# raphaelsulzer/PixelsPointsPolygons

Hardware: NVIDIA B200
Metric: pillar_encode_tiles_per_sec (higher is better)
Workload: dtype f16 operands, f32 accumulate, f32 in/out

## Files before the change

### pixelspointspolygons_b200/csrc/pfn.cu

```cuda
#include <cuda_fp16.h>

#include "p3p_internal.cuh"

namespace p3p {

#ifdef P3P_TIMELINE
constexpr int kTlCtas = 4, kTlRoles = 12, kTlIters = 96, kTlStamps = 4;
__device__ long long g_pfn_tl[kTlCtas][kTlRoles][kTlIters][kTlStamps];
__device__ __forceinline__ void ptl(int role, long long it, int k) {
    if ((threadIdx.x & 31) == 0 && blockIdx.x < kTlCtas && it < kTlIters) g_pfn_tl[blockIdx.x][role][it][k] = clock64();
}
#define PTL(role, it, k) ptl(role, it, k)
extern "C" int p3p_debug_pfn_timeline(long long* host) {
    return (int)cudaMemcpyFromSymbol(host, g_pfn_tl, sizeof(g_pfn_tl));
}
#else
#define PTL(role, it, k)
#endif

void make_blob_layout(int C, BlobLayout* out) {
    BlobLayout l;
    l.C = C;
    l.Cpad = (C + 127) / 128 * 128;
    l.MT = l.Cpad / 128;
    size_t off = 0;
    auto take = [&](size_t bytes) {
        size_t o = off;
        off += (bytes + 1023) / 1024 * 1024;
        return o;
    };
    l.off_header = take(64);
    l.off_front = take(10 * 32 * 4);
    l.off_w0 = take(32 * 8 * 4);
    l.off_b0 = take(32 * 4);
    l.off_w1 = take((size_t)l.Cpad * 64 * 4);
    l.off_b1 = take((size_t)l.Cpad * 4);
    l.off_a1 = take((size_t)l.Cpad * 128);
    l.off_a2 = take((size_t)l.Cpad * 128);
    l.total_bytes = off;
    *out = l;
}

namespace {

__global__ void pfn_prepare_kernel(p3p_pfn_params p, int precision, char* blob, BlobLayout bl) {
    const int tid = blockIdx.x * blockDim.x + threadIdx.x;
    const int nthreads = gridDim.x * blockDim.x;
    int* header = reinterpret_cast<int*>(blob + bl.off_header);
    float* front = reinterpret_cast<float*>(blob + bl.off_front);
    float* w0 = reinterpret_cast<float*>(blob + bl.off_w0);
    float* b0 = reinterpret_cast<float*>(blob + bl.off_b0);
    float* w1 = reinterpret_cast<float*>(blob + bl.off_w1);
    float* b1 = reinterpret_cast<float*>(blob + bl.off_b1);
    if (tid == 0) {
        header[0] = kBlobMagic; header[1] = precision; header[2] = bl.C; header[3] = bl.Cpad; header[4] = p.center_alias;
    }
    for (int k = tid; k < kC0; k += nthreads) {
        const float a = p.norm0_weight[k] / sqrtf(p.norm0_var[k] + p.eps);
        const float sh = p.norm0_bias[k] - p.norm0_mean[k] * a;
        float w[8];
        for (int i = 0; i < 8; ++i) {
            w[i] = a * p.linear0_weight[k * 8 + i];
            w0[k * 8 + i] = w[i];
        }
        b0[k] = sh;
        front[0 * 32 + k] = w[0] + w[3] + w[6];
        front[1 * 32 + k] = w[1] + w[4] + w[7];
        front[2 * 32 + k] = w[2] + w[5];
        front[3 * 32 + k] = p.center_alias ? 0.f : w[0];
        front[4 * 32 + k] = p.center_alias ? 0.f : w[1];
        front[5 * 32 + k] = w[3];
        front[6 * 32 + k] = w[4];
        front[7 * 32 + k] = w[5];
        front[8 * 32 + k] = sh;
        front[9 * 32 + k] = fmaxf(sh, 0.f);
        if (precision == P3P_PRECISION_TF32) {
            const float up = 1.0f + 0x1p-12f;
            for (int r = 0; r < 10; ++r) front[r * 32 + k] *= up;
        }
    }
    const bool tf32 = (precision != P3P_PRECISION_BF16 && precision != P3P_PRECISION_FP16);
    for (int c = tid; c < bl.Cpad; c += nthreads) {
        float a = 0.f, sh = 0.f;
        if (c < bl.C) {
            a = p.norm1_weight[c] / sqrtf(p.norm1_var[c] + p.eps);
            sh = p.norm1_bias[c] - p.norm1_mean[c] * a;
        }
        b1[c] = sh;
        const int t = c >> 7, r = c & 127;
        for (int j = 0; j < 64; ++j) {
            const float v = (c < bl.C) ? a * p.linear1_weight[c * 64 + j] : 0.f;
            w1[c * 64 + j] = v;
            const int k = j & 31;
            char* tile = blob + (j < 32 ? bl.off_a1 : bl.off_a2);
            if (tf32) {
                const size_t o = (size_t)t * 16384 + (size_t)(r >> 3) * 1024 + (size_t)(r & 7) * 128 +
                                 (size_t)(((k >> 2) ^ (r & 7)) * 16) + (size_t)(k & 3) * 4;
                *reinterpret_cast<uint32_t*>(tile + o) = to_tf32(v);
            } else {
                const size_t o = (size_t)t * 8192 + (size_t)(r >> 3) * 512 + (size_t)(r & 7) * 64 +
                                 (size_t)(((k >> 3) ^ ((r >> 1) & 3)) * 16) + (size_t)(k & 7) * 2;
                *reinterpret_cast<unsigned short*>(tile + o) = (precision == P3P_PRECISION_FP16)
                                                                   ? __half_as_ushort(__float2half_rn(v))
                                                                   : (unsigned short)(pack_bf16(v, 0.f) & 0xFFFF);
            }
        }
    }
}

__device__ __forceinline__ void store_scalar(const PfnArgs& a, int64_t idx, float v) {
    if (a.out_dtype == P3P_DTYPE_F32) {
        static_cast<float*>(a.out)[idx] = v;
    } else {
        static_cast<unsigned short*>(a.out)[idx] = to_16bit(v, a.out_dtype);
    }
}
__device__ __forceinline__ int64_t out_index(const PfnArgs& a, int64_t item, int b, int cell, int c) {
    if (a.item_mode == kItemsCanvas && a.out_layout == P3P_LAYOUT_NCHW)
        return ((int64_t)b * a.c_total + a.c_offset + c) * a.items_per_tile + cell;
    return item * a.row_stride + a.row_offset + c;
}
__device__ __forceinline__ void store_item(const PfnArgs& a, int64_t item, int b, int cell, int c, float v) {
    if (a.token_rows) {
        static_cast<float*>(a.out)[((int64_t)b * a.token_rows + 1 + cell) * a.bl.C + c] = v + a.pos_embed[(int64_t)(1 + cell) * a.bl.C + c];
        return;
    }
    store_scalar(a, out_index(a, item, b, cell, c), v);
}

constexpr int kSimtMaxThreads = 512;
constexpr int kHStride = 36;

template <bool kHoist>
__global__ void __launch_bounds__(kSimtMaxThreads) pfn_simt_kernel(PfnArgs a) {
    extern __shared__ __align__(16) float smem_f[];
    float* H = smem_f;
    float* w0s = H + (size_t)(a.g.M + 1) * kHStride;
    float* b0s = w0s + 256;
    int* red = reinterpret_cast<int*>(b0s + 32);
    int* hmax_bits = red + 96;

    const int tid = threadIdx.x, lane = tid & 31, w = tid >> 5, nthreads = blockDim.x, nwarps = nthreads >> 5;
    const float* w0g = reinterpret_cast<const float*>(a.blob + a.bl.off_w0);
    const float* b0g = reinterpret_cast<const float*>(a.blob + a.bl.off_b0);
    const float* w1g = reinterpret_cast<const float*>(a.blob + a.bl.off_w1);
    const float* b1g = reinterpret_cast<const float*>(a.blob + a.bl.off_b1);
    const int alias = reinterpret_cast<const int*>(a.blob + a.bl.off_header)[4];
    for (int i = tid; i < 256; i += nthreads) w0s[i] = w0g[i];
    if (tid < 32) b0s[tid] = b0g[tid];
    const int C = a.bl.C, M = a.g.M;
    float wa[32], wb[32], b1c = 0.f;
    if (kHoist) {
        const int c = tid < C ? tid : 0;
        b1c = b1g[c];
#pragma unroll
        for (int k = 0; k < 32; ++k) { wa[k] = w1g[(size_t)c * 64 + k]; wb[k] = w1g[(size_t)c * 64 + 32 + k]; }
    }
    __syncthreads();

    for (int64_t item = blockIdx.x; item < a.num_items; item += gridDim.x) {
        const Item it = fetch_item(a, item);
        if (!it.valid) {
            if (a.item_mode == kItemsCanvas)
                for (int c = tid; c < C; c += nthreads) store_item(a, item, it.b, it.cell, c, 0.f);
            continue;
        }
        const float4* slot = item_slots(a, it);
        const int n = it.n;
        int sl[3] = {0, 0, 0}, sh[3] = {0, 0, 0};
        for (int r = tid; r < n; r += nthreads) {
            const float4 p = slot[r];
            int lo, hi;
            fix_split(p.x, a.g.fix_scale, lo, hi); sl[0] += lo; sh[0] += hi;
            fix_split(p.y, a.g.fix_scale, lo, hi); sl[1] += lo; sh[1] += hi;
            fix_split(p.z, a.g.fix_scale, lo, hi); sl[2] += lo; sh[2] += hi;
        }
#pragma unroll
        for (int i = 0; i < 3; ++i) {
            sl[i] = __reduce_add_sync(0xffffffffu, sl[i]);
            sh[i] = __reduce_add_sync(0xffffffffu, sh[i]);
            if (lane == 0) { red[w * 6 + i] = sl[i]; red[w * 6 + 3 + i] = sh[i]; }
        }
        if (tid < 32) hmax_bits[tid] = 0;
        __syncthreads();
        int tl[3] = {0, 0, 0}, th[3] = {0, 0, 0};
        for (int ww = 0; ww < nwarps; ++ww) {
#pragma unroll
            for (int i = 0; i < 3; ++i) { tl[i] += red[ww * 6 + i]; th[i] += red[ww * 6 + 3 + i]; }
        }
        const float fn = (float)n;
        const float mx = fix_mean(tl[0], th[0], a.g.fix_inv, fn);
        const float my = fix_mean(tl[1], th[1], a.g.fix_inv, fn);
        const float mz = fix_mean(tl[2], th[2], a.g.fix_inv, fn);

        float hm[32];
#pragma unroll
        for (int k = 0; k < 32; ++k) hm[k] = 0.f;
        bool any_row = false;
        for (int r = tid; r < n; r += nthreads) {
            any_row = true;
            const float4 p = slot[r];
            float d[8];
            const float xc = p.x - it.ctr_x, yc = p.y - it.ctr_y;
            d[0] = alias ? xc : p.x; d[1] = alias ? yc : p.y; d[2] = p.z;
            d[3] = p.x - mx; d[4] = p.y - my; d[5] = p.z - mz;
            d[6] = xc; d[7] = yc;
            float* hrow = H + (size_t)r * kHStride;
#pragma unroll
            for (int k = 0; k < 32; ++k) {
                float acc = 0.f;
#pragma unroll
                for (int i = 0; i < 8; ++i) acc = __fmaf_rn(w0s[k * 8 + i], d[i], acc);
                const float h = fmaxf(acc + b0s[k], 0.f);
                hrow[k] = h;
                hm[k] = fmaxf(hm[k], h);
            }
        }
        if (__any_sync(0xffffffffu, any_row)) {
#pragma unroll
            for (int k = 0; k < 32; ++k) {
                const float v = warp_max_f32(hm[k]);
                if (lane == 0) atomicMax(&hmax_bits[k], __float_as_int(v));
            }
        }
        if (n < M && tid < 32) {
            const float hp = fmaxf(b0s[tid], 0.f);
            H[(size_t)n * kHStride + tid] = hp;
            atomicMax(&hmax_bits[tid], __float_as_int(hp));
        }
        __syncthreads();
        const int rows = n + (n < M ? 1 : 0);
        if (kHoist) {
            if (tid < C) {
                float g = b1c;
#pragma unroll
                for (int k = 0; k < 32; ++k) g = __fmaf_rn(wb[k], __int_as_float(hmax_bits[k]), g);
                float best = -INFINITY;
                for (int r = 0; r < rows; ++r) {
                    const float4* hr = reinterpret_cast<const float4*>(H + (size_t)r * kHStride);
                    float acc = 0.f;
#pragma unroll
                    for (int k4 = 0; k4 < 8; ++k4) {
                        const float4 h = hr[k4];
                        acc = __fmaf_rn(wa[k4 * 4 + 0], h.x, acc);
                        acc = __fmaf_rn(wa[k4 * 4 + 1], h.y, acc);
                        acc = __fmaf_rn(wa[k4 * 4 + 2], h.z, acc);
                        acc = __fmaf_rn(wa[k4 * 4 + 3], h.w, acc);
                    }
                    best = fmaxf(best, acc);
                }
                store_item(a, item, it.b, it.cell, tid, fmaxf(best + g, 0.f));
            }
        } else {
            for (int c = tid; c < C; c += nthreads) {
                float g = b1g[c];
#pragma unroll
                for (int k = 0; k < 32; ++k) {
                    wa[k] = w1g[(size_t)c * 64 + k];
                    g = __fmaf_rn(w1g[(size_t)c * 64 + 32 + k], __int_as_float(hmax_bits[k]), g);
                }
                float best = -INFINITY;
                for (int r = 0; r < rows; ++r) {
                    const float4* hr = reinterpret_cast<const float4*>(H + (size_t)r * kHStride);
                    float acc = 0.f;
#pragma unroll
                    for (int k4 = 0; k4 < 8; ++k4) {
                        const float4 h = hr[k4];
                        acc = __fmaf_rn(wa[k4 * 4 + 0], h.x, acc);
                        acc = __fmaf_rn(wa[k4 * 4 + 1], h.y, acc);
                        acc = __fmaf_rn(wa[k4 * 4 + 2], h.z, acc);
                        acc = __fmaf_rn(wa[k4 * 4 + 3], h.w, acc);
                    }
                    best = fmaxf(best, acc);
                }
                store_item(a, item, it.b, it.cell, c, fmaxf(best + g, 0.f));
            }
        }
        __syncthreads();
    }
}

__global__ void cls_rows_kernel(PfnArgs a, const float* __restrict__ cls_token) {
    const int C = a.bl.C;
    const int64_t total = (int64_t)a.B * C;
    for (int64_t i = (int64_t)blockIdx.x * blockDim.x + threadIdx.x; i < total; i += (int64_t)gridDim.x * blockDim.x) {
        const int64_t b = i / C;
        const int c = (int)(i - b * C);
        static_cast<float*>(a.out)[b * a.token_rows * C + c] = cls_token[c] + a.pos_embed[c];
    }
}

__global__ void zero_lidar_kernel(PfnArgs a) {
    const int C = a.bl.C;
    const int64_t total = a.num_items * C;
    for (int64_t i = (int64_t)blockIdx.x * blockDim.x + threadIdx.x; i < total; i += (int64_t)gridDim.x * blockDim.x) {
        int64_t idx;
        if (a.out_layout == P3P_LAYOUT_NCHW) {
            const int64_t per_tile = (int64_t)C * a.items_per_tile;
            const int64_t b = i / per_tile, rem = i - b * per_tile;
            idx = (b * a.c_total + a.c_offset) * a.items_per_tile + rem;
        } else {
            const int64_t item = i / C;
            idx = item * a.row_stride + a.row_offset + (i - item * C);
        }
        store_scalar(a, idx, 0.f);
    }
}

constexpr int kNF = 8;
constexpr int kMmaWarps = 4;
constexpr int kEpiWarp0 = kMmaWarps + kNF;
constexpr int kEpiGroups = 3;
constexpr int kTcThreads = 32 * (kEpiWarp0 + 4 * kEpiGroups);

constexpr int kRegMma = 40, kRegFront = 104, kRegEpi = 72;
static_assert(4 * kRegMma + 8 * kRegFront + 12 * kRegEpi <= 24 * 80, "register pool of the launch exceeded");
constexpr int kUnit = 8;
constexpr int kPairsPerUnit = kUnit / 2;
constexpr int kTiles = 3;
constexpr int kAccCols = 64;
constexpr int kAccStages = 2;
constexpr int kGCol0 = kTiles * kAccStages * kAccCols;
constexpr int kGSlotCols = kTiles * 16;
constexpr int kValidRing = 64;
constexpr int kStageRows = 128;

template <int kPrec>
struct TcCfg {
    static constexpr bool kTf32 = (kPrec == P3P_PRECISION_TF32);
    static constexpr int kFmt = kTf32 ? 2 : (kPrec == P3P_PRECISION_BF16 ? 1 : 0);
    static constexpr int RB = kTf32 ? 128 : 64;
    static constexpr int kATile = 128 * RB;
    static constexpr int kHStage = kStageRows * RB;
    static constexpr int kGStage = 16 * RB;
    static constexpr uint32_t kLayout = kTf32 ? 2u : 4u;
    static constexpr uint32_t kSBO = 8 * RB;
    static constexpr int kKSteps = kTf32 ? 4 : 2;
    static constexpr int kNS = kTf32 ? 4 : 8;
    static constexpr size_t kSmemOperands = (size_t)6 * kATile + (size_t)kNS * kHStage + 2 * (size_t)kGStage;
    static constexpr size_t kSmemFloats = 10 * 32 + 384 + kNF * 128 * 4;
    static constexpr size_t kSmemBytes = kSmemOperands + kSmemFloats * 4 + (2 * kNS + 2 * kTiles * kAccStages + 4 * kTiles + 2 + 2) * 8 + 16 + 2 * kNF * 4 + 2 * kValidRing + 4 * kEpiGroups * kUnit * 32 * 4 + 2 * kNF * 4 * 4 + 2 * kNF * 32 * 4;
};


template <int kPrec>
__device__ __forceinline__ uint32_t pack_relu16(float lo, float hi) {
    uint32_t r;
    if constexpr (kPrec == P3P_PRECISION_BF16)
        asm("cvt.rn.relu.bf16x2.f32 %0, %1, %2;" : "=r"(r) : "f"(hi), "f"(lo));
    else
        asm("cvt.rn.relu.f16x2.f32 %0, %1, %2;" : "=r"(r) : "f"(hi), "f"(lo));
    return r;
}
template <int kPrec>
__device__ __forceinline__ uint32_t max16x2(uint32_t a, uint32_t b) {
    uint32_t r;
    if constexpr (kPrec == P3P_PRECISION_BF16)
        asm("max.bf16x2 %0, %1, %2;" : "=r"(r) : "r"(a), "r"(b));
    else
        asm("max.f16x2 %0, %1, %2;" : "=r"(r) : "r"(a), "r"(b));
    return r;
}
__device__ __forceinline__ void sts128(uint32_t addr, uint32_t a, uint32_t b, uint32_t c, uint32_t d) {
    asm volatile("st.shared.v4.b32 [%0], {%1, %2, %3, %4};" ::"r"(addr), "r"(a), "r"(b), "r"(c), "r"(d) : "memory");
}
__device__ __forceinline__ void cp_async16(uint32_t dst, const void* src, uint32_t src_bytes) {
    asm volatile("cp.async.ca.shared.global [%0], [%1], 16, %2;" ::"r"(dst), "l"(src), "r"(src_bytes) : "memory");
}
template <int kRegs>
__device__ __forceinline__ void setmaxnreg_inc() { asm volatile("setmaxnreg.inc.sync.aligned.u32 %0;" ::"n"(kRegs)); }
template <int kRegs>
__device__ __forceinline__ void setmaxnreg_dec() { asm volatile("setmaxnreg.dec.sync.aligned.u32 %0;" ::"n"(kRegs)); }
__device__ __forceinline__ void cp_async4(uint32_t dst, const void* src) {
    asm volatile("cp.async.ca.shared.global [%0], [%1], 4;" ::"r"(dst), "l"(src) : "memory");
}
__device__ __forceinline__ void cp_async_wait_all() { asm volatile("cp.async.wait_all;" ::: "memory"); }

struct ItemWalk {
    int b, r, ipt, db, dr;
    __device__ __forceinline__ void init(int item, int delta, int items_per_tile) {
        ipt = items_per_tile;
        b = item / ipt; r = item - b * ipt;
        db = delta / ipt; dr = delta - db * ipt;
    }
    __device__ __forceinline__ void step() {
        b += db; r += dr;
        if (r >= ipt) { r -= ipt; ++b; }
    }
};

__device__ __forceinline__ void tmem_ld8_wait(uint32_t taddr, float (&v)[8]) {
    asm volatile(
        "tcgen05.ld.sync.aligned.32x32b.x8.b32 {%0,%1,%2,%3,%4,%5,%6,%7}, [%8];\n"
        "tcgen05.wait::ld.sync.aligned;\n"
        : "=f"(v[0]), "=f"(v[1]), "=f"(v[2]), "=f"(v[3]), "=f"(v[4]), "=f"(v[5]), "=f"(v[6]), "=f"(v[7])
        : "r"(taddr)
        : "memory");
}
__device__ __forceinline__ float max16(const float (&v)[16]) {
    float r[5];
#pragma unroll
    for (int i = 0; i < 5; ++i) r[i] = fmax3(v[3 * i], v[3 * i + 1], v[3 * i + 2]);
    return fmax3(fmax3(r[0], r[1], r[2]), fmaxf(r[3], r[4]), v[15]);
}
__device__ __forceinline__ float max16_with(float prev, const float (&v)[16]) {
    const float r0 = fmax3(prev, v[0], v[1]), r1 = fmax3(v[2], v[3], v[4]), r2 = fmax3(v[5], v[6], v[7]);
    const float r3 = fmax3(v[8], v[9], v[10]), r4 = fmax3(v[11], v[12], v[13]);
    return fmax3(fmax3(r0, r1, r2), fmax3(r3, r4, v[14]), v[15]);
}
template <int kPrec, int kMode>
__global__ void __launch_bounds__(kTcThreads, 1) pfn_tc_kernel(PfnArgs a) {
    using Cfg = TcCfg<kPrec>;
    constexpr bool kTf32 = Cfg::kTf32;
    constexpr int kNS = Cfg::kNS;
    extern __shared__ __align__(1024) unsigned char smem_dyn[];
    unsigned char* base = smem_dyn;
    unsigned char* sA1 = base;
    unsigned char* sA2 = sA1 + 3 * Cfg::kATile;
    unsigned char* sH = sA2 + 3 * Cfg::kATile;
    unsigned char* sG = sH + kNS * Cfg::kHStage;
    float* sFront = reinterpret_cast<float*>(sG + 2 * Cfg::kGStage);
    float* sB1 = sFront + 10 * 32;
    float4* sPts = reinterpret_cast<float4*>(sB1 + 384);
    uint64_t* bars = reinterpret_cast<uint64_t*>(sPts + kNF * 128);
    uint64_t* h_full = bars;
    uint64_t* h_empty = bars + kNS;
    uint64_t* t_full = bars + 2 * kNS;
    uint64_t* t_empty = t_full + kTiles * kAccStages;
    uint64_t* gt_full = t_empty + kTiles * kAccStages;
    uint64_t* gt_empty = gt_full + 2 * kTiles;
    uint64_t* g_empty = gt_empty + 2 * kTiles;
    uint32_t* tmem_slot = reinterpret_cast<uint32_t*>(g_empty + 2);
    int* sDesc = reinterpret_cast<int*>(tmem_slot + 2);
    unsigned char* sValid = reinterpret_cast<unsigned char*>(sDesc + 2 * kNF);
    float* sRmax = reinterpret_cast<float*>(sValid + 2 * kValidRing);
    int* sBlkSum = reinterpret_cast<int*>(sRmax + 4 * kEpiGroups * kUnit * 32);
    uint32_t* sBlkMax = reinterpret_cast<uint32_t*>(sBlkSum + 2 * kNF * 4);

    const int tid = threadIdx.x, warp = tid >> 5, lane = tid & 31;
    const int MT = a.bl.MT;
    const int total_items = (int)a.num_items;
    const int bs = (kMode == 0) ? a.blk_shift : 0;
    const int num_units = ((total_items << bs) + kUnit - 1) / kUnit;
    const int my_units = (num_units > (int)blockIdx.x) ? (num_units - (int)blockIdx.x + (int)gridDim.x - 1) / (int)gridDim.x : 0;
    const int my_pairs = my_units * kPairsPerUnit;
    const bool canvas = (kMode != 0) || (a.item_mode == kItemsCanvas);

    if ((smem_u32(smem_dyn) & 1023u) != 0u) __trap();
    if (warp == 0) tmem_alloc(tmem_slot, 512);
    if (tid == 32) {
        for (int i = 0; i < kNS; ++i) { mbar_init(&h_full[i], 2); mbar_init(&h_empty[i], (uint32_t)MT); }
        for (int i = 0; i < kTiles * kAccStages; ++i) { mbar_init(&t_full[i], 1); mbar_init(&t_empty[i], 128); }
        for (int i = 0; i < 2 * kTiles; ++i) { mbar_init(&gt_full[i], 1); mbar_init(&gt_empty[i], 128); }
        mbar_init(&g_empty[0], (uint32_t)MT); mbar_init(&g_empty[1], (uint32_t)MT);
        fence_mbar_init();
    }
    {
        const uint4* g1 = reinterpret_cast<const uint4*>(a.blob + a.bl.off_a1);
        const uint4* g2 = reinterpret_cast<const uint4*>(a.blob + a.bl.off_a2);
        const int nvec = MT * Cfg::kATile / 16;
        for (int i = tid; i < nvec; i += kTcThreads) {
            reinterpret_cast<uint4*>(sA1)[i] = g1[i];
            reinterpret_cast<uint4*>(sA2)[i] = g2[i];
        }
        for (int i = tid; i < 2 * Cfg::kGStage / 16; i += kTcThreads) reinterpret_cast<uint4*>(sG)[i] = make_uint4(0, 0, 0, 0);
        const float* fg = reinterpret_cast<const float*>(a.blob + a.bl.off_front);
        const float* b1g = reinterpret_cast<const float*>(a.blob + a.bl.off_b1);
        for (int i = tid; i < 10 * 32; i += kTcThreads) sFront[i] = fg[i];
        for (int i = tid; i < 384; i += kTcThreads) sB1[i] = (i < a.bl.Cpad) ? b1g[i] : 0.f;
    }
    fence_async_smem();
    tc_fence_before();
    __syncthreads();
    tc_fence_after();
    const uint32_t tmem_base = *tmem_slot;
    asm volatile("griddepcontrol.wait;" ::: "memory");

    if (warp < kMmaWarps) {
        setmaxnreg_dec<kRegMma>();
        const int m = warp;
        if (m < MT) {
            const bool leader = elect_one();
            const uint32_t idesc_main = make_idesc(Cfg::kFmt, 128, kAccCols);
            const uint32_t idesc_g = make_idesc(Cfg::kFmt, 128, 16);
            const uint32_t desc_hi = (Cfg::kSBO >> 4) | (1u << 14) | (Cfg::kLayout << 29);
            const uint32_t a1_lo = ((smem_u32(sA1) + (uint32_t)(m * Cfg::kATile)) >> 4) | (1u << 16);
            const uint32_t a2_lo = ((smem_u32(sA2) + (uint32_t)(m * Cfg::kATile)) >> 4) | (1u << 16);
            const uint32_t h_lo = (smem_u32(sH) >> 4) | (1u << 16), g_lo = (smem_u32(sG) >> 4) | (1u << 16);
            const uint32_t d_tile = tmem_base + (uint32_t)(m * kAccStages * kAccCols);
            const uint32_t d_g = tmem_base + (uint32_t)(kGCol0 + m * 16);
            uint64_t* tf = t_full + m * kAccStages;
            uint64_t* te = t_empty + m * kAccStages;
            int st = 0;
            uint32_t use = 0;
            for (int p = 0; p < my_pairs; ++p) {
                mbar_wait(&h_full[st], use & 1);
                if (m == 0) PTL(0, p, 0);
                const uint32_t hs_lo = h_lo + (uint32_t)st * (Cfg::kHStage >> 4);
#pragma unroll
                for (int s = 0; s < kAccStages; ++s) {
                    mbar_wait(&te[s], ((uint32_t)p & 1u) ^ 1u);
                    if (m == 0 && s == 0) PTL(0, p, 1);
                    tc_fence_after();
                    if (leader) {
                        const uint32_t b_lo = hs_lo + (uint32_t)(s * ((64 * Cfg::RB) >> 4));
#pragma unroll
                        for (int k = 0; k < Cfg::kKSteps; ++k)
                            tc_mma<kTf32>(d_tile + (uint32_t)(s * kAccCols), ((uint64_t)desc_hi << 32) | (a1_lo + (uint32_t)(k * 2)),
                                          ((uint64_t)desc_hi << 32) | (b_lo + (uint32_t)(k * 2)), idesc_main, k > 0);
                        tc_commit(&tf[s]);
                    }
                    __syncwarp();
                }
                if (leader) tc_commit(&h_empty[st]);
                __syncwarp();
                if (m == 0) PTL(0, p, 2);
                if (++st == kNS) { st = 0; ++use; }
                if ((p & (kPairsPerUnit - 1)) == kPairsPerUnit - 1) {
                    const uint32_t j = (uint32_t)p / kPairsPerUnit, slot = j & 1u;
                    mbar_wait(&gt_empty[m * 2 + slot], ((j >> 1) & 1u) ^ 1u);
                    tc_fence_after();
                    if (leader) {
                        const uint32_t gs_lo = g_lo + slot * (Cfg::kGStage >> 4);
#pragma unroll
                        for (int k = 0; k < Cfg::kKSteps; ++k)
                            tc_mma<kTf32>(d_g + slot * kGSlotCols, ((uint64_t)desc_hi << 32) | (a2_lo + (uint32_t)(k * 2)),
                                          ((uint64_t)desc_hi << 32) | (gs_lo + (uint32_t)(k * 2)), idesc_g, k > 0);
                        tc_commit(&gt_full[m * 2 + slot]);
                        tc_commit(&g_empty[slot]);
                    }
                    __syncwarp();
                }
            }
        }
    } else if (warp < kEpiWarp0) {
        setmaxnreg_inc<kRegFront>();
        const int fw = warp - kMmaWarps, half = fw & 1, pr = fw >> 1;
        const int o = lane & 3, pt = lane >> 2;
        float2 ux[4], uy[4], uz[4];
#pragma unroll
        for (int i = 0; i < 4; ++i) {
            ux[i] = *reinterpret_cast<const float2*>(sFront + 0 * 32 + 8 * o + 2 * i);
            uy[i] = *reinterpret_cast<const float2*>(sFront + 1 * 32 + 8 * o + 2 * i);
            uz[i] = *reinterpret_cast<const float2*>(sFront + 2 * 32 + 8 * o + 2 * i);
        }
        const float* kc = sFront + 8 * o;
        const float k_cx = sFront[3 * 32 + lane], k_cy = sFront[4 * 32 + lane], k_mx = sFront[5 * 32 + lane];
        const float k_my = sFront[6 * 32 + lane], k_mz = sFront[7 * 32 + lane], k_b0 = sFront[8 * 32 + lane];
        float4* pbuf = sPts + fw * 128;
        const uint32_t pbuf_sa = smem_u32(pbuf);
        uint32_t row_off[2];
        if constexpr (kTf32) {
            row_off[0] = (uint32_t)(half * 64 + pt) * Cfg::RB + (uint32_t)(((2 * o) ^ pt) * 16);
            row_off[1] = (uint32_t)(half * 64 + pt) * Cfg::RB + (uint32_t)(((2 * o + 1) ^ pt) * 16);
        } else {
            row_off[0] = (uint32_t)(half * 64 + pt) * Cfg::RB + (uint32_t)((o ^ ((pt >> 1) & 3)) * 16);
            row_off[1] = 0;
        }
        const uint32_t g_off0 = (uint32_t)fw * Cfg::RB + (uint32_t)(kTf32 ? (((2 * o) ^ (fw & 7)) * 16) : ((o ^ ((fw >> 1) & 3)) * 16));
        const uint32_t g_off1 = (uint32_t)fw * Cfg::RB + (uint32_t)(((2 * o + 1) ^ (fw & 7)) * 16);
        const float inv_nx = 1.0f / (float)a.g.nx;
        const int kblk = fw & ((1 << bs) - 1), row0 = kblk * 64;
        auto item_of = [&](int j) -> int {
            const int it = (((int)blockIdx.x + j * (int)gridDim.x) * kUnit + fw) >> bs;
            return (j < my_units && it < total_items) ? it : total_items;
        };
        auto block_rows = [&](const Item& it) -> int {
            const int r = it.n - row0;
            return r < 0 ? 0 : (r > 64 ? 64 : r);
        };
        auto block_valid = [&](const Item& it) -> bool {
            return it.valid && (bs == 0 || it.n > row0 || (it.n == row0 && it.n < a.g.M));
        };
        int* my_desc = sDesc + 2 * fw;
        const uint32_t my_desc_sa = smem_u32(my_desc);
        auto prefetch_desc = [&](int j) {
            const int item = item_of(j);
            if (lane == 0) {
                if (canvas && item < total_items) cp_async4(my_desc_sa + 4u * (uint32_t)(j & 1), a.ws.cell_desc + item);
                else my_desc[j & 1] = -1;
            }
        };
        ItemWalk wk;
        wk.init(item_of(0) < total_items ? item_of(0) : 0, ((int)gridDim.x * kUnit) >> bs, a.items_per_tile);
        auto decode = [&](int j, int d) -> Item {
            Item it;
            if (!canvas) {
                it = fetch_item(a, item_of(j));
            } else {
                it.valid = d >= 0 ? 1 : 0;
                it.b = wk.b; it.cell = wk.r;
                it.key = d & 0xFFFF; it.n = d >> 16;
                const int cy = __float2int_rz(((float)wk.r + 0.5f) * inv_nx), cx = wk.r - cy * a.g.nx;
                it.ctr_x = __fmaf_rn((float)cx, a.g.vx, a.g.x_off);
                it.ctr_y = __fmaf_rn((float)cy, a.g.vy, a.g.y_off);
            }
            wk.step();
            return it;
        };
        auto prefetch_points = [&](const Item& it, int set) {
            if (block_valid(it)) {
                const float4* sl = item_slots(a, it) + row0;
                const int nr = block_rows(it);
                const uint32_t dst = pbuf_sa + (uint32_t)set * 1024u + (uint32_t)lane * 16u;
                cp_async16(dst, sl + lane, lane < nr ? 16u : 0u);
                cp_async16(dst + 512u, sl + lane + 32, lane + 32 < nr ? 16u : 0u);
            }
        };
        prefetch_desc(0);
        cp_async_wait_all();
        __syncwarp();
        Item it_cur = decode(0, my_desc[0]);
        __syncwarp();
        prefetch_points(it_cur, 0);
        prefetch_desc(1);
        for (int j = 0; j < my_units; ++j) {
            const Item it = it_cur;
            cp_async_wait_all();
            __syncwarp();
            it_cur = decode(j + 1, my_desc[(j + 1) & 1]);
            __syncwarp();
            prefetch_points(it_cur, (j + 1) & 1);
            prefetch_desc(j + 2);

            const int p = j * kPairsPerUnit + pr, st = p % kNS;
            const uint32_t use = (uint32_t)(p / kNS);
            PTL(1 + fw, j, 0);
            mbar_wait(&h_empty[st], (use & 1u) ^ 1u);
            mbar_wait(&g_empty[j & 1], (((uint32_t)j >> 1) & 1u) ^ 1u);
            PTL(1 + fw, j, 1);
            const uint32_t gslot_sa = smem_u32(sG) + (uint32_t)(j & 1) * Cfg::kGStage;
            const bool bvalid = block_valid(it);
            const float4* P = pbuf + (j & 1) * 64;
            uint32_t hm[8] = {0u, 0u, 0u, 0u, 0u, 0u, 0u, 0u};
            int sx = 0, sy = 0, sz = 0;
            if (bvalid) {
                const float4 s0 = P[lane], s1 = P[lane + 32];
                const float fs = a.g.fix2_scale;
                sx = __reduce_add_sync(0xffffffffu, __float2int_rn(s0.x * fs) + __float2int_rn(s1.x * fs));
                sy = __reduce_add_sync(0xffffffffu, __float2int_rn(s0.y * fs) + __float2int_rn(s1.y * fs));
                sz = __reduce_add_sync(0xffffffffu, __float2int_rn(s0.z * fs) + __float2int_rn(s1.z * fs));
            }
            if (bs) {
                int* mine = sBlkSum + ((j & 1) * kNF + fw) * 4;
                if (lane == 0) { mine[0] = sx; mine[1] = sy; mine[2] = sz; }
                asm volatile("bar.sync %0, %1;" ::"r"(1 + (fw >> bs)), "r"(32 << bs) : "memory");
                const int* first = sBlkSum + ((j & 1) * kNF + (fw - kblk)) * 4;
                sx = sy = sz = 0;
                for (int k = 0; k < (1 << bs); ++k) { sx += first[4 * k]; sy += first[4 * k + 1]; sz += first[4 * k + 2]; }
            }
            if (bvalid) {
                const int n = block_rows(it);
                const int n_all = it.n;
                float mpx, mpy, mz;
                {
                    const float wn = __fdividef(a.g.fix2_inv, (float)n_all);
                    mpx = (float)sx * wn - it.ctr_x;
                    mpy = (float)sy * wn - it.ctr_y;
                    mz = (float)sz * wn;
                }
                float qx[8], qy[8], qz[8];
#pragma unroll
                for (int i = 0; i < 8; ++i) {
                    const float4 q = P[pt + 8 * i];
                    qx[i] = q.x - it.ctr_x; qy[i] = q.y - it.ctr_y; qz[i] = q.z;
                }
                float2 kap[4];
                {
                    float kl = __fmaf_rn(k_cx, it.ctr_x, k_b0);
                    kl = __fmaf_rn(k_cy, it.ctr_y, kl);
                    kl = __fmaf_rn(k_mx, -mpx, kl);
                    kl = __fmaf_rn(k_my, -mpy, kl);
                    kl = __fmaf_rn(k_mz, -mz, kl);
#pragma unroll
                    for (int i = 0; i < 4; ++i)
                        kap[i] = make_float2(__shfl_sync(0xffffffffu, kl, 8 * o + 2 * i), __shfl_sync(0xffffffffu, kl, 8 * o + 2 * i + 1));
                }
                const uint32_t stage_sa = smem_u32(sH) + (uint32_t)st * Cfg::kHStage;
                if constexpr (kTf32) {
                    float hp[8], mx8[8];
                    if (n_all < a.g.M || n == 64) {
#pragma unroll
                        for (int c = 0; c < 8; ++c) hp[c] = kc[9 * 32 + c];
                    } else {
                        const float4 q0 = P[0];
                        const float x0 = q0.x - it.ctr_x, y0 = q0.y - it.ctr_y, z0 = q0.z;
#pragma unroll
                        for (int c = 0; c < 4; ++c) {
                            const float2 v = ffma2(ux[c], make_float2(x0, x0), ffma2(uy[c], make_float2(y0, y0), ffma2(uz[c], make_float2(z0, z0), kap[c])));
                            hp[2 * c] = fmaxf(v.x, 0.f); hp[2 * c + 1] = fmaxf(v.y, 0.f);
                        }
                    }
#pragma unroll
                    for (int c = 0; c < 8; ++c) mx8[c] = (n < 64) ? hp[c] : 0.f;
#pragma unroll
                    for (int i = 0; i < 8; ++i) {
                        float h[8];
#pragma unroll
                        for (int c = 0; c < 4; ++c) {
                            const float2 v = ffma2(ux[c], make_float2(qx[i], qx[i]), ffma2(uy[c], make_float2(qy[i], qy[i]), ffma2(uz[c], make_float2(qz[i], qz[i]), kap[c])));
                            h[2 * c] = fmaxf(v.x, 0.f); h[2 * c + 1] = fmaxf(v.y, 0.f);
                        }
                        if (pt + 8 * i >= n) {
#pragma unroll
                            for (int c = 0; c < 8; ++c) h[c] = hp[c];
                        }
#pragma unroll
                        for (int c = 0; c < 8; ++c) mx8[c] = fmaxf(mx8[c], h[c]);
                        sts128(stage_sa + row_off[0] + (uint32_t)i * (8u * Cfg::RB), __float_as_uint(h[0]), __float_as_uint(h[1]), __float_as_uint(h[2]), __float_as_uint(h[3]));
                        sts128(stage_sa + row_off[1] + (uint32_t)i * (8u * Cfg::RB), __float_as_uint(h[4]), __float_as_uint(h[5]), __float_as_uint(h[6]), __float_as_uint(h[7]));
                    }
#pragma unroll
                    for (int off = 4; off < 32; off <<= 1) {
#pragma unroll
                        for (int c = 0; c < 8; ++c) mx8[c] = fmaxf(mx8[c], __shfl_xor_sync(0xffffffffu, mx8[c], off));
                    }
                    if (bs) {
#pragma unroll
                        for (int c = 0; c < 8; ++c) hm[c] = __float_as_uint(mx8[c]);
                    } else if (pt == 0) {
                        sts128(gslot_sa + g_off0, __float_as_uint(mx8[0]), __float_as_uint(mx8[1]), __float_as_uint(mx8[2]), __float_as_uint(mx8[3]));
                        sts128(gslot_sa + g_off1, __float_as_uint(mx8[4]), __float_as_uint(mx8[5]), __float_as_uint(mx8[6]), __float_as_uint(mx8[7]));
                    }
                } else {
                    uint32_t mm[4] = {0u, 0u, 0u, 0u};
                    if (n == 64) {
#pragma unroll
                        for (int i = 0; i < 8; ++i) {
                            uint32_t h[4];
#pragma unroll
                            for (int c = 0; c < 4; ++c) {
                                const float2 v = ffma2(ux[c], make_float2(qx[i], qx[i]), ffma2(uy[c], make_float2(qy[i], qy[i]), ffma2(uz[c], make_float2(qz[i], qz[i]), kap[c])));
                                h[c] = pack_relu16<kPrec>(v.x, v.y);
                                mm[c] = max16x2<kPrec>(mm[c], h[c]);
                            }
                            sts128(stage_sa + row_off[0] + (uint32_t)i * (8u * Cfg::RB), h[0], h[1], h[2], h[3]);
                        }
                    } else {
                        uint32_t hp[4];
                        if (n_all < a.g.M) {
#pragma unroll
                            for (int c = 0; c < 4; ++c) hp[c] = pack_relu16<kPrec>(kc[9 * 32 + 2 * c], kc[9 * 32 + 2 * c + 1]);
                        } else {
                            const float4 q0 = P[0];
                            const float x0 = q0.x - it.ctr_x, y0 = q0.y - it.ctr_y, z0 = q0.z;
#pragma unroll
                            for (int c = 0; c < 4; ++c) {
                                const float2 v = ffma2(ux[c], make_float2(x0, x0), ffma2(uy[c], make_float2(y0, y0), ffma2(uz[c], make_float2(z0, z0), kap[c])));
                                hp[c] = pack_relu16<kPrec>(v.x, v.y);
                            }
                        }
#pragma unroll
                        for (int i = 0; i < 8; ++i) {
                            uint32_t h[4];
#pragma unroll
                            for (int c = 0; c < 4; ++c) {
                                const float2 v = ffma2(ux[c], make_float2(qx[i], qx[i]), ffma2(uy[c], make_float2(qy[i], qy[i]), ffma2(uz[c], make_float2(qz[i], qz[i]), kap[c])));
                                h[c] = pack_relu16<kPrec>(v.x, v.y);
                                if (pt + 8 * i >= n) h[c] = hp[c];
                                mm[c] = max16x2<kPrec>(mm[c], h[c]);
                            }
                            sts128(stage_sa + row_off[0] + (uint32_t)i * (8u * Cfg::RB), h[0], h[1], h[2], h[3]);
                        }
                    }
#pragma unroll
                    for (int off = 4; off < 32; off <<= 1) {
#pragma unroll
                        for (int c = 0; c < 4; ++c) mm[c] = max16x2<kPrec>(mm[c], __shfl_xor_sync(0xffffffffu, mm[c], off));
                    }
                    if (bs) {
#pragma unroll
                        for (int c = 0; c < 4; ++c) hm[c] = mm[c];
                    } else if (pt == 0) {
                        sts128(gslot_sa + g_off0, mm[0], mm[1], mm[2], mm[3]);
                    }
                }
            }
            if (bs) {
                constexpr int kW = kTf32 ? 8 : 4;
                uint32_t* mine = sBlkMax + ((j & 1) * kNF + fw) * 32 + kW * o;
                if (pt == 0) {
#pragma unroll
                    for (int c = 0; c < kW; ++c) mine[c] = hm[c];
                }
                asm volatile("bar.sync %0, %1;" ::"r"(1 + (fw >> bs)), "r"(32 << bs) : "memory");
                if (pt == 0) {
                    const uint32_t* first = sBlkMax + ((j & 1) * kNF + (fw - kblk)) * 32 + kW * o;
                    for (int k = 0; k < (1 << bs); ++k) {
#pragma unroll
                        for (int c = 0; c < kW; ++c) {
                            const uint32_t v = first[32 * k + c];
                            if constexpr (kTf32) hm[c] = __float_as_uint(fmaxf(__uint_as_float(hm[c]), __uint_as_float(v)));
                            else hm[c] = max16x2<kPrec>(hm[c], v);
                        }
                    }
                    sts128(gslot_sa + g_off0, hm[0], hm[1], hm[2], hm[3]);
                    if constexpr (kTf32) sts128(gslot_sa + g_off1, hm[4], hm[5], hm[6], hm[7]);
                }
            }
            if (lane == 0) sValid[(p & (kValidRing - 1)) * 2 + half] = (unsigned char)bvalid;
            fence_async_smem();
            __syncwarp();
            PTL(1 + fw, j, 2);
            if (lane == 0) mbar_arrive(&h_full[st]);
        }
    } else {
        setmaxnreg_dec<kRegEpi>();
        const int g = (warp - kEpiWarp0) >> 2;
        const int quad = warp & 3;
        const bool nchw = (kMode == 2) || (kMode == 0 && canvas && (a.out_layout == P3P_LAYOUT_NCHW));
        const bool f32 = (kMode == 2) || (kMode == 3) || (a.out_dtype == P3P_DTYPE_F32);
        const int C = a.bl.C, ipt = a.items_per_tile;
        const bool fast = (kMode != 0) || (bs == 0 && canvas && (total_items % kUnit == 0) && (ipt % kUnit == 0) && a.token_rows == 0);
        const bool tokens = (kMode == 3);
        const uint32_t tlane = tmem_base + ((uint32_t)(quad * 32) << 16);
        const int cl = quad * 32 + lane;
        float b1v[3];
#pragma unroll
        for (int mm = 0; mm < 3; ++mm) b1v[mm] = sB1[mm * 128 + cl];
        ItemWalk wu;
        wu.init((((int)blockIdx.x * kUnit) >> bs) < total_items ? (((int)blockIdx.x * kUnit) >> bs) : 0, ((int)gridDim.x * kUnit) >> bs, ipt);
        int unit_item0 = ((int)blockIdx.x * kUnit) >> bs;
        const int m = g;
        const float bb = (m == 0) ? b1v[0] : ((m == 1) ? b1v[1] : b1v[2]);
        const int c = m * 128 + cl;
        const uint32_t taddr = tlane + (uint32_t)(g * kAccStages * kAccCols);
        const uint32_t gaddr = tlane + (uint32_t)(kGCol0 + g * 16);
        const uint32_t tf_sa = opaque(smem_u32(t_full + g * kAccStages));
        const uint32_t te_sa = opaque(smem_u32(t_empty + g * kAccStages));
        const uint32_t gtf_sa = opaque(smem_u32(gt_full + 2 * g)), gte_sa = opaque(smem_u32(gt_empty + 2 * g));
        int jn = 0;
        uint32_t ready = 0;
        float va[16], vb[16];
        const uint32_t rmax_sa = opaque(smem_u32(sRmax + (warp - kEpiWarp0) * (kUnit * 32) + lane));
        const uint32_t valid_sa = opaque(smem_u32(sValid));
        const uint32_t taddr_o = opaque(taddr);
        const int64_t rs = a.row_stride;
        const int64_t rows_first = (int64_t)blockIdx.x * kUnit * rs + a.row_offset + c;
        float* rows_dst = static_cast<float*>(a.out) + rows_first;
        unsigned short* rows_dst16 = static_cast<unsigned short*>(a.out) + rows_first;
        const int64_t rows_step = (int64_t)gridDim.x * kUnit * rs;
        auto unit_tail = [&](int j, int ub, int ur, int item0) {
            float rmax[kUnit];
#pragma unroll
            for (int i = 0; i < kUnit; ++i) rmax[i] = lds_f32(rmax_sa + (uint32_t)(i * 128));
            float gv[8];
            mbar_wait_sa(gtf_sa + 8u * ((uint32_t)j & 1u), ((uint32_t)j >> 1) & 1u);
            tc_fence_after();
            tmem_ld8_wait(gaddr + (uint32_t)((j & 1) * kGSlotCols), gv);
            tc_fence_before();
            mbar_arrive_sa(gte_sa + 8u * ((uint32_t)j & 1u));
            const uint2 vv = lds_u32x2(valid_sa + (uint32_t)(((j * kPairsPerUnit) & (kValidRing - 1)) * 2));
            float ob[kUnit];
#pragma unroll
            for (int i = 0; i < kUnit; ++i) {
                const unsigned word = i < 4 ? vv.x : vv.y;
                const bool v = ((word >> (8 * (i & 3))) & 0xFFu) != 0;
                ob[i] = v ? fmaxf(rmax[i] + (gv[i] + bb), 0.f) : 0.f;
            }
            if (c < C) {
                if (tokens) {
                    const int64_t row = (int64_t)ub * a.token_rows + 1 + ur;
                    float* dst = static_cast<float*>(a.out) + row * C + c;
                    const float* pe = a.pos_embed + (int64_t)(1 + ur) * C + c;
#pragma unroll
                    for (int i = 0; i < kUnit; ++i) dst[(int64_t)i * C] = ob[i] + __ldg(pe + (int64_t)i * C);
                } else if (fast) {
                    if (nchw) {
                        const int64_t i0 = ((int64_t)ub * a.c_total + a.c_offset + c) * ipt + ur;
                        if (f32) {
                            float4* dst = reinterpret_cast<float4*>(static_cast<float*>(a.out) + i0);
                            dst[0] = make_float4(ob[0], ob[1], ob[2], ob[3]);
                            dst[1] = make_float4(ob[4], ob[5], ob[6], ob[7]);
                        } else {
                            const int dt = a.out_dtype;
                            *reinterpret_cast<uint4*>(static_cast<unsigned short*>(a.out) + i0) =
                                make_uint4((uint32_t)to_16bit(ob[0], dt) | ((uint32_t)to_16bit(ob[1], dt) << 16), (uint32_t)to_16bit(ob[2], dt) | ((uint32_t)to_16bit(ob[3], dt) << 16),
                                           (uint32_t)to_16bit(ob[4], dt) | ((uint32_t)to_16bit(ob[5], dt) << 16), (uint32_t)to_16bit(ob[6], dt) | ((uint32_t)to_16bit(ob[7], dt) << 16));
                        }
                    } else if (f32) {
                        float* dst = rows_dst;
#pragma unroll
                        for (int i = 0; i < kUnit; ++i) { *dst = ob[i]; dst += rs; }
                    } else {
                        unsigned short* dst = rows_dst16;
#pragma unroll
                        for (int i = 0; i < kUnit; ++i) { *dst = to_16bit(ob[i], a.out_dtype); dst += rs; }
                    }
                } else {
                    if (bs) {
                        const int bpp = 1 << bs;
#pragma unroll
                        for (int i = 0; i < kUnit; ++i) {
                            const unsigned word = i < 4 ? vv.x : vv.y;
                            const bool v = ((word >> (8 * (i & 3))) & 0xFFu) != 0;
                            ob[i] = v ? rmax[i] + (gv[i] + bb) : -INFINITY;
                        }
#pragma unroll
                        for (int i = 0; i < kUnit; ++i) {
                            if ((i & (bpp - 1)) == 0) {
                                float mval = ob[i];
#pragma unroll
                                for (int k = 1; k < kUnit; ++k)
                                    if (k < bpp && i + k < kUnit) mval = fmaxf(mval, ob[i + k]);
                                ob[i >> bs] = mval == -INFINITY ? -INFINITY : fmaxf(mval, 0.f);
                            }
                        }
                    }
                    int bi = ub, ri = ur;
#pragma unroll
                    for (int i = 0; i < kUnit; ++i) {
                        if (bs && i >= (kUnit >> bs)) break;
                        const int item = item0 + i;
                        const unsigned word = i < 4 ? vv.x : vv.y;
                        bool v = ((word >> (8 * (i & 3))) & 0xFFu) != 0;
                        if (bs) { v = ob[i] != -INFINITY; if (!v) ob[i] = 0.f; }
                        if (item < total_items && (v || canvas)) {
                            if (a.token_rows) {
                                static_cast<float*>(a.out)[((int64_t)bi * a.token_rows + 1 + ri) * C + c] =
                                    ob[i] + a.pos_embed[(int64_t)(1 + ri) * C + c];
                            } else {
                                const int64_t idx = nchw ? ((int64_t)bi * a.c_total + a.c_offset + c) * ipt + ri : (int64_t)item * rs + a.row_offset + c;
                                store_scalar(a, idx, ob[i]);
                            }
                        }
                        if (++ri >= ipt) { ri = 0; ++bi; }
                    }
                }
            }
            rows_dst += rows_step;
            rows_dst16 += rows_step;
            if (quad == 0) PTL(9 + g, 8 * j + 7, 3);
        };
        const int my_units_g = (g < MT) ? my_units : 0;
        for (int j = 0; j < my_units_g; ++j) {
            const int ub = wu.b, ur = wu.r;
            const int item0 = unit_item0;
            wu.step();
            unit_item0 += ((int)gridDim.x * kUnit) >> bs;
#pragma unroll
            for (int pr = 0; pr < kPairsPerUnit; ++pr) {
#pragma unroll
                for (int s = 0; s < kAccStages; ++s, ++jn) {
                    const uint32_t tph = (uint32_t)pr & 1u;
                    if (quad == 0) PTL(9 + g, jn, 0);
                    if (!ready) mbar_wait_sa(tf_sa + 8u * s, tph);
                    tc_fence_after();
                    tmem_ld16_issue(taddr_o + (uint32_t)(s * kAccCols), va);
                    if (quad == 0) PTL(9 + g, jn, 1);
                    tmem_ld_wait16(va);
                    tmem_ld16_issue(taddr_o + (uint32_t)(s * kAccCols + 16), vb);
                    ready = (2 * pr + s + 1 < kUnit || j + 1 < my_units_g) ? mbar_test_sa(tf_sa + 8u * (s ^ 1), (uint32_t)((2 * pr + s + 1) >> 1) & 1u) : 0u;
                    const float r0 = max16(va);
                    tmem_ld_wait16(vb);
                    tmem_ld16_issue(taddr_o + (uint32_t)(s * kAccCols + 32), va);
                    const float r1 = max16_with(r0, vb);
                    tmem_ld_wait16(va);
                    tmem_ld16_issue(taddr_o + (uint32_t)(s * kAccCols + 48), vb);
                    const float r2 = max16_with(r1, va);
                    tmem_ld_wait16(vb);
                    tc_fence_before();
                    mbar_arrive_sa(te_sa + 8u * s);
                    sts_f32(rmax_sa + (uint32_t)((2 * pr + s) * 128), max16_with(r2, vb));
                    if (quad == 0) PTL(9 + g, jn, 2);
                }
            }
            unit_tail(j, ub, ur, item0);
        }
    }
    tc_fence_before();
    __syncthreads();
    if (warp == 0) tmem_dealloc(tmem_base, 512);
}

}

int launch_pfn_prepare(const p3p_pfn_params* p, int precision, char* blob, const BlobLayout& bl, cudaStream_t st) {
    pfn_prepare_kernel<<<4, 128, 0, st>>>(*p, precision, blob, bl);
    P3P_CUDA_CHECK(cudaGetLastError());
    return P3P_OK;
}

int launch_pfn_simt(const PfnArgs& a, cudaStream_t st) {
    if (a.num_items <= 0) return P3P_OK;
    if (a.num_items > 0x7fffffff - 64) return fail(P3P_ERR_UNSUPPORTED, "%lld work items exceed the 32-bit item index", (long long)a.num_items);
    const size_t smem = ((size_t)(a.g.M + 1) * kHStride + 256 + 32 + 96 + 32) * sizeof(float);
    P3P_CUDA_CHECK(cudaFuncSetAttribute(pfn_simt_kernel<true>, cudaFuncAttributeMaxDynamicSharedMemorySize, 200 * 1024));
    P3P_CUDA_CHECK(cudaFuncSetAttribute(pfn_simt_kernel<false>, cudaFuncAttributeMaxDynamicSharedMemorySize, 200 * 1024));
    const int sms = device_sm_count();
    const bool hoist = a.bl.C <= kSimtMaxThreads;
    const int threads = hoist ? (a.bl.C + 31) / 32 * 32 : kSimtMaxThreads;
    int64_t grid = (int64_t)sms * (hoist ? (threads <= 256 ? 4 : 2) : 2);
    if (grid > a.num_items) grid = a.num_items;
    if (hoist)
        pfn_simt_kernel<true><<<(unsigned)grid, threads, smem, st>>>(a);
    else
        pfn_simt_kernel<false><<<(unsigned)grid, threads, smem, st>>>(a);
    P3P_CUDA_CHECK(cudaGetLastError());
    return P3P_OK;
}

int launch_cls_rows(const PfnArgs& a, const float* cls_token, cudaStream_t st) {
    if (a.B <= 0) return P3P_OK;
    const int64_t total = (int64_t)a.B * a.bl.C;
    cls_rows_kernel<<<(unsigned)((total + 255) / 256 < 1024 ? (total + 255) / 256 : 1024), 256, 0, st>>>(a, cls_token);
    P3P_CUDA_CHECK(cudaGetLastError());
    return P3P_OK;
}

int launch_zero_lidar(const PfnArgs& a, cudaStream_t st) {
    if (a.num_items <= 0) return P3P_OK;
    zero_lidar_kernel<<<device_sm_count() * 4, 256, 0, st>>>(a);
    P3P_CUDA_CHECK(cudaGetLastError());
    return P3P_OK;
}

int launch_pfn_tc(const PfnArgs& a_in, int precision, cudaStream_t st) {
    if (a_in.num_items <= 0) return P3P_OK;
    if (a_in.num_items > 0x7fffffff - 64) return fail(P3P_ERR_UNSUPPORTED, "%lld work items exceed the 32-bit item index", (long long)a_in.num_items);
    PfnArgs a = a_in;
    a.blk_shift = 0;
    while ((64 << a.blk_shift) < a.g.M) ++a.blk_shift;
    if ((a.num_items << a.blk_shift) > 0x7fffffff - 64) return fail(P3P_ERR_UNSUPPORTED, "too many row blocks for the 32-bit item index");
    const int64_t units = ((a.num_items << a.blk_shift) + kUnit - 1) / kUnit;
    int64_t grid = device_sm_count();
    if (grid > units) grid = units;
    int mode = 0;
    if (a.blk_shift == 0 && a.item_mode == kItemsCanvas && a.num_items % kUnit == 0 && a.items_per_tile % kUnit == 0) {
        if (a.token_rows) mode = a.out_dtype == P3P_DTYPE_F32 ? 3 : 0;
        else if (a.out_layout == P3P_LAYOUT_NCHW) mode = a.out_dtype == P3P_DTYPE_F32 ? 2 : 0;
        else mode = 1;
    }
    cudaLaunchAttribute attr[1];
    attr[0].id = cudaLaunchAttributeProgrammaticStreamSerialization;
    attr[0].val.programmaticStreamSerializationAllowed = 1;
    cudaLaunchConfig_t cfg = {};
    cfg.gridDim = dim3((unsigned)grid);
    cfg.blockDim = dim3(kTcThreads);
    cfg.stream = st;
    cfg.attrs = attr;
    cfg.numAttrs = 1;
#define P3P_LAUNCH_TC(PREC, MODE)                      \
    do {                                               \
        cfg.dynamicSmemBytes = TcCfg<PREC>::kSmemBytes; \
        P3P_CUDA_CHECK(cudaFuncSetAttribute(pfn_tc_kernel<PREC, MODE>, cudaFuncAttributeMaxDynamicSharedMemorySize, \
                                            (int)TcCfg<PREC>::kSmemBytes));  \
        P3P_CUDA_CHECK(cudaLaunchKernelEx(&cfg, pfn_tc_kernel<PREC, MODE>, a)); \
    } while (0)
#define P3P_LAUNCH_TC_MODES(PREC)                         \
    do {                                                  \
        if (mode == 1) P3P_LAUNCH_TC(PREC, 1);            \
        else if (mode == 2) P3P_LAUNCH_TC(PREC, 2);       \
        else if (mode == 3) P3P_LAUNCH_TC(PREC, 3);       \
        else P3P_LAUNCH_TC(PREC, 0);                      \
    } while (0)
    if (precision == P3P_PRECISION_TF32) P3P_LAUNCH_TC_MODES(P3P_PRECISION_TF32);
    else if (precision == P3P_PRECISION_BF16) P3P_LAUNCH_TC_MODES(P3P_PRECISION_BF16);
    else P3P_LAUNCH_TC_MODES(P3P_PRECISION_FP16);
#undef P3P_LAUNCH_TC_MODES
#undef P3P_LAUNCH_TC
    P3P_CUDA_CHECK(cudaGetLastError());
    return P3P_OK;
}

}
```

Before: 305,000.

## Fold G-tile MMA into the last accumulator stage and drop gt barriers

Moves the per-unit G MMA so it is issued before the final accumulator stage of each unit, ordered through the existing t_full commit, and removes the dedicated gt_full/gt_empty mbarrier pair. The epilogue now issues the 8-column G TMEM load alongside the last stage's accumulator load instead of waiting on a separate barrier in the unit tail. This removes one barrier wait/arrive round trip per unit on both the MMA and epilogue sides. The trade-off is that G slot reuse now relies on the t_empty ordering and double-buffered slots rather than an explicit empty barrier, which is a subtle correctness dependency.

```diff
diff --git a/pixelspointspolygons_b200/csrc/pfn.cu b/pixelspointspolygons_b200/csrc/pfn.cu
--- a/pixelspointspolygons_b200/csrc/pfn.cu
+++ b/pixelspointspolygons_b200/csrc/pfn.cu
@@ -339,7 +339,7 @@
     static constexpr int kNS = kTf32 ? 4 : 8;
     static constexpr size_t kSmemOperands = (size_t)6 * kATile + (size_t)kNS * kHStage + 2 * (size_t)kGStage;
     static constexpr size_t kSmemFloats = 10 * 32 + 384 + kNF * 128 * 4;
-    static constexpr size_t kSmemBytes = kSmemOperands + kSmemFloats * 4 + (2 * kNS + 2 * kTiles * kAccStages + 4 * kTiles + 2 + 2) * 8 + 16 + 2 * kNF * 4 + 2 * kValidRing + 4 * kEpiGroups * kUnit * 32 * 4 + 2 * kNF * 4 * 4 + 2 * kNF * 32 * 4;
+    static constexpr size_t kSmemBytes = kSmemOperands + kSmemFloats * 4 + (2 * kNS + 2 * kTiles * kAccStages + 2 + 2) * 8 + 16 + 2 * kNF * 4 + 2 * kValidRing + 4 * kEpiGroups * kUnit * 32 * 4 + 2 * kNF * 4 * 4 + 2 * kNF * 32 * 4;
 };
 
 
@@ -389,13 +389,17 @@
     }
 };
 
-__device__ __forceinline__ void tmem_ld8_wait(uint32_t taddr, float (&v)[8]) {
-    asm volatile(
-        "tcgen05.ld.sync.aligned.32x32b.x8.b32 {%0,%1,%2,%3,%4,%5,%6,%7}, [%8];\n"
-        "tcgen05.wait::ld.sync.aligned;\n"
-        : "=f"(v[0]), "=f"(v[1]), "=f"(v[2]), "=f"(v[3]), "=f"(v[4]), "=f"(v[5]), "=f"(v[6]), "=f"(v[7])
-        : "r"(taddr)
-        : "memory");
+__device__ __forceinline__ void tmem_ld8_issue(uint32_t taddr, float (&v)[8]) {
+    asm volatile("tcgen05.ld.sync.aligned.32x32b.x8.b32 {%0,%1,%2,%3,%4,%5,%6,%7}, [%8];\n"
+                 : "=f"(v[0]), "=f"(v[1]), "=f"(v[2]), "=f"(v[3]), "=f"(v[4]), "=f"(v[5]), "=f"(v[6]), "=f"(v[7])
+                 : "r"(taddr)
+                 : "memory");
+}
+__device__ __forceinline__ void tmem_ld_wait8(float (&v)[8]) {
+    asm volatile("tcgen05.wait::ld.sync.aligned;\n"
+                 : "+f"(v[0]), "+f"(v[1]), "+f"(v[2]), "+f"(v[3]), "+f"(v[4]), "+f"(v[5]), "+f"(v[6]), "+f"(v[7])
+                 :
+                 : "memory");
 }
 __device__ __forceinline__ float max16(const float (&v)[16]) {
     float r[5];
@@ -427,9 +431,7 @@
     uint64_t* h_empty = bars + kNS;
     uint64_t* t_full = bars + 2 * kNS;
     uint64_t* t_empty = t_full + kTiles * kAccStages;
-    uint64_t* gt_full = t_empty + kTiles * kAccStages;
-    uint64_t* gt_empty = gt_full + 2 * kTiles;
-    uint64_t* g_empty = gt_empty + 2 * kTiles;
+    uint64_t* g_empty = t_empty + kTiles * kAccStages;
     uint32_t* tmem_slot = reinterpret_cast<uint32_t*>(g_empty + 2);
     int* sDesc = reinterpret_cast<int*>(tmem_slot + 2);
     unsigned char* sValid = reinterpret_cast<unsigned char*>(sDesc + 2 * kNF);
@@ -451,7 +453,6 @@
     if (tid == 32) {
         for (int i = 0; i < kNS; ++i) { mbar_init(&h_full[i], 2); mbar_init(&h_empty[i], (uint32_t)MT); }
         for (int i = 0; i < kTiles * kAccStages; ++i) { mbar_init(&t_full[i], 1); mbar_init(&t_empty[i], 128); }
-        for (int i = 0; i < 2 * kTiles; ++i) { mbar_init(&gt_full[i], 1); mbar_init(&gt_empty[i], 128); }
         mbar_init(&g_empty[0], (uint32_t)MT); mbar_init(&g_empty[1], (uint32_t)MT);
         fence_mbar_init();
     }
@@ -499,6 +500,18 @@
                 const uint32_t hs_lo = h_lo + (uint32_t)st * (Cfg::kHStage >> 4);
 #pragma unroll
                 for (int s = 0; s < kAccStages; ++s) {
+                    if (s == 1 && (p & (kPairsPerUnit - 1)) == kPairsPerUnit - 1) {
+                        const uint32_t j = (uint32_t)p / kPairsPerUnit, slot = j & 1u;
+                        if (leader) {
+                            const uint32_t gs_lo = g_lo + slot * (Cfg::kGStage >> 4);
+#pragma unroll
+                            for (int k = 0; k < Cfg::kKSteps; ++k)
+                                tc_mma<kTf32>(d_g + slot * kGSlotCols, ((uint64_t)desc_hi << 32) | (a2_lo + (uint32_t)(k * 2)),
+                                              ((uint64_t)desc_hi << 32) | (gs_lo + (uint32_t)(k * 2)), idesc_g, k > 0);
+                            tc_commit(&g_empty[slot]);
+                        }
+                        __syncwarp();
+                    }
                     mbar_wait(&te[s], ((uint32_t)p & 1u) ^ 1u);
                     if (m == 0 && s == 0) PTL(0, p, 1);
                     tc_fence_after();
@@ -516,21 +529,6 @@
                 __syncwarp();
                 if (m == 0) PTL(0, p, 2);
                 if (++st == kNS) { st = 0; ++use; }
-                if ((p & (kPairsPerUnit - 1)) == kPairsPerUnit - 1) {
-                    const uint32_t j = (uint32_t)p / kPairsPerUnit, slot = j & 1u;
-                    mbar_wait(&gt_empty[m * 2 + slot], ((j >> 1) & 1u) ^ 1u);
-                    tc_fence_after();
-                    if (leader) {
-                        const uint32_t gs_lo = g_lo + slot * (Cfg::kGStage >> 4);
-#pragma unroll
-                        for (int k = 0; k < Cfg::kKSteps; ++k)
-                            tc_mma<kTf32>(d_g + slot * kGSlotCols, ((uint64_t)desc_hi << 32) | (a2_lo + (uint32_t)(k * 2)),
-                                          ((uint64_t)desc_hi << 32) | (gs_lo + (uint32_t)(k * 2)), idesc_g, k > 0);
-                        tc_commit(&gt_full[m * 2 + slot]);
-                        tc_commit(&g_empty[slot]);
-                    }
-                    __syncwarp();
-                }
             }
         }
     } else if (warp < kEpiWarp0) {
@@ -825,13 +823,12 @@
         const float bb = (m == 0) ? b1v[0] : ((m == 1) ? b1v[1] : b1v[2]);
         const int c = m * 128 + cl;
         const uint32_t taddr = tlane + (uint32_t)(g * kAccStages * kAccCols);
-        const uint32_t gaddr = tlane + (uint32_t)(kGCol0 + g * 16);
         const uint32_t tf_sa = opaque(smem_u32(t_full + g * kAccStages));
         const uint32_t te_sa = opaque(smem_u32(t_empty + g * kAccStages));
-        const uint32_t gtf_sa = opaque(smem_u32(gt_full + 2 * g)), gte_sa = opaque(smem_u32(gt_empty + 2 * g));
         int jn = 0;
         uint32_t ready = 0;
         float va[16], vb[16];
+        float gv[8];
         const uint32_t rmax_sa = opaque(smem_u32(sRmax + (warp - kEpiWarp0) * (kUnit * 32) + lane));
         const uint32_t valid_sa = opaque(smem_u32(sValid));
         const uint32_t taddr_o = opaque(taddr);
@@ -844,12 +841,6 @@
             float rmax[kUnit];
 #pragma unroll
             for (int i = 0; i < kUnit; ++i) rmax[i] = lds_f32(rmax_sa + (uint32_t)(i * 128));
-            float gv[8];
-            mbar_wait_sa(gtf_sa + 8u * ((uint32_t)j & 1u), ((uint32_t)j >> 1) & 1u);
-            tc_fence_after();
-            tmem_ld8_wait(gaddr + (uint32_t)((j & 1) * kGSlotCols), gv);
-            tc_fence_before();
-            mbar_arrive_sa(gte_sa + 8u * ((uint32_t)j & 1u));
             const uint2 vv = lds_u32x2(valid_sa + (uint32_t)(((j * kPairsPerUnit) & (kValidRing - 1)) * 2));
             float ob[kUnit];
 #pragma unroll
@@ -947,8 +938,12 @@
                     if (!ready) mbar_wait_sa(tf_sa + 8u * s, tph);
                     tc_fence_after();
                     tmem_ld16_issue(taddr_o + (uint32_t)(s * kAccCols), va);
+                    const bool last = (2 * pr + s == kUnit - 1);
+                    if (last)
+                        tmem_ld8_issue(taddr_o + (uint32_t)(kGCol0 + g * 16 - g * kAccStages * kAccCols + (j & 1) * kGSlotCols), gv);
                     if (quad == 0) PTL(9 + g, jn, 1);
                     tmem_ld_wait16(va);
+                    if (last) tmem_ld_wait8(gv);
                     tmem_ld16_issue(taddr_o + (uint32_t)(s * kAccCols + 16), vb);
                     ready = (2 * pr + s + 1 < kUnit || j + 1 < my_units_g) ? mbar_test_sa(tf_sa + 8u * (s ^ 1), (uint32_t)((2 * pr + s + 1) >> 1) & 1u) : 0u;
                     const float r0 = max16(va);
```

Result: faster. 308,600 (median of 6 runs) (+1.2%).
